# zju3dv/BoxDreamer

Hardware: AMD Instinct MI355X
Metric: poses/s/GPU (5-ref, 224×224, bf16); heatmap max-abs err vs CPU ref (higher is better)
Workload: dtype f16 + e4m3 corrections (BETR q, k columns: f16)

## Files before the change

boxdreamer_amd/csrc/attention.hip:

```cpp
#include "bd_common.h"
#include <type_traits>

#ifdef BD_ATTN_PROBE
__device__ unsigned* bd_attn_probe_buf = nullptr;
extern "C" int bd_attn_probe_set(void* buf) { return (int)hipMemcpyToSymbol(HIP_SYMBOL(bd_attn_probe_buf), &buf, sizeof(buf)); }
#define AP(idx) { const unsigned long long t__ = __builtin_amdgcn_s_memtime(); if ((idx) < 64) probe_ts = (lane == (idx)) ? (unsigned)t__ : probe_ts; }
#else
#define AP(idx) {}
#endif

namespace {

struct AttnArgs {
    const void* qkv; int64_t qkv_plane;
    void* out; int64_t out_plane;
    int batch, seq, heads;
    float scale_log2e;
    const int32_t* q_view;
    int q_len;
    int q_off;
    int out_rows;
};

constexpr int KT = 64;

__device__ __forceinline__ int vswz(int d) { return ((d >> 1) ^ (d >> 4)) & 7; }

__device__ __forceinline__ unsigned pack_lo16(unsigned a, unsigned b) { return __builtin_amdgcn_perm(b, a, 0x05040100u); }
__device__ __forceinline__ unsigned pack_hi16(unsigned a, unsigned b) { return __builtin_amdgcn_perm(b, a, 0x07060302u); }

template <class T, int NS, int HD, int NW, int OUTMODE = 0>
__global__ __launch_bounds__(NW * 64, NS == 1 && HD == 64 ? 3 : 2) void attn_kernel(const AttnArgs p) {
    bd_saturating_conversions();
    typedef typename Op16<T>::vec8 vec8;
    constexpr int NT = NW * 64;
    constexpr int DCH = HD / 8;
    constexpr int KSTRIDE = HD * 2 + 16;
    constexpr int K_BYTES = KT * KSTRIDE;
    constexpr int V_BYTES = HD * 128;
    constexpr int PLANE_BYTES = K_BYTES + V_BYTES;
    constexpr int KCH = KT * DCH;
    constexpr int KCPT = (KCH + NT - 1) / NT;
    constexpr int VMT = (KT / 4) * DCH;
    static_assert(VMT <= NT, "one V micro-tile per thread");
    constexpr int QB = NW * 32;
    constexpr int DM = HD / 32;
    constexpr int KS = HD / 16;
    constexpr int BUF_BYTES = NS * PLANE_BYTES;
    constexpr int NBUF = NS == 1 ? 2 : 1;
    __shared__ __attribute__((aligned(16))) unsigned char lds[NBUF * BUF_BYTES];

    const int tid = threadIdx.x, lane = tid & 63, wid = tid >> 6;
#ifdef BD_ATTN_PROBE
    unsigned probe_ts = 0;
    AP(60)
#endif
    const int lq = lane & 31, lh = lane >> 5;
    const int seq = p.seq, heads = p.heads;
    const int q_len = p.q_len;
    const int nqb = (q_len + QB - 1) / QB;

    int wg;
    {
        const int nwg = gridDim.x, bid = blockIdx.x, xcd = bid & 7, q = nwg >> 3, r = nwg & 7;
        wg = (xcd < r ? xcd * (q + 1) : r * (q + 1) + (xcd - r) * q) + (bid >> 3);
    }
    const int qb = wg % nqb;
    const int bh = wg / nqb;
    const int head = bh % heads, b = bh / heads;

    const int ld = 3 * heads * HD;
    const T* base = (const T*)p.qkv + (int64_t)b * seq * ld + head * HD;
    const T* qbase = base;
    const T* kbase = base + heads * HD;
    const T* vbase = base + 2 * heads * HD;
    const int64_t plane = p.qkv_plane;

    const int q0 = qb * QB + wid * 32;
    const int qbase_row = p.q_view ? p.q_view[b] * q_len : p.q_off;
    int qrow = q0 + lq; qrow = (qrow < q_len ? qrow : q_len - 1) + qbase_row;
    vec8 qf[NS][KS];
#pragma unroll
    for (int s = 0; s < NS; ++s)
#pragma unroll
        for (int ks = 0; ks < KS; ++ks)
            qf[s][ks] = as_vec8<T>(*(const u128*)(qbase + s * plane + (unsigned)(qrow * ld + ks * 16 + lh * 8)));

    int kc_row[KCPT], kc_col[KCPT];
    unsigned kc_off[KCPT];
#pragma unroll
    for (int i = 0; i < KCPT; ++i) {
        const int c = tid + NT * i;
        kc_row[i] = c / DCH;
        kc_col[i] = c % DCH;
        kc_off[i] = (unsigned)(kc_row[i] * ld + kc_col[i] * 8);
    }
    const int vm_kq = tid / DCH, vm_dc = tid % DCH;
    const bool vm_active = tid < VMT;
    const unsigned vm_off = (unsigned)(vm_kq * 4 * ld + vm_dc * 8);
    const bool ragged = (seq % KT) != 0;
    int vdst;
    {
        const int g = vm_kq >> 2, qi = vm_kq & 3;
        const int qp = (qi == 1) ? 2 : (qi == 2 ? 1 : qi);
        vdst = ((g * 2 + (qp >> 1)) << 4) | ((qp & 1) << 3);
    }

    u128 rk[NS][KCPT], rv[NS][4];
    __amdgpu_buffer_rsrc_t rsrc[NS];
    {
        const int bytes = __builtin_amdgcn_readfirstlane(seq * ld * (int)sizeof(T));
#pragma unroll
        for (int s = 0; s < NS; ++s) {
            const uintptr_t a = (uintptr_t)(base + s * plane);
            const unsigned lo = __builtin_amdgcn_readfirstlane((unsigned)a), hi = __builtin_amdgcn_readfirstlane((unsigned)(a >> 32));
            rsrc[s] = __builtin_amdgcn_make_buffer_rsrc((void*)(((uintptr_t)hi << 32) | lo), 0, bytes, 0x00020000);
        }
    }
    const int row_bytes = __builtin_amdgcn_readfirstlane(ld * (int)sizeof(T));
    int k_voff[KCPT];
#pragma unroll
    for (int i = 0; i < KCPT; ++i) k_voff[i] = ((int)kc_off[i] + heads * HD) * (int)sizeof(T);
    const int v_voff = ((int)vm_off + 2 * heads * HD) * (int)sizeof(T);
#define LOAD_TILE(kt)                                                                         \
    _Pragma("unroll") for (int s = 0; s < NS; ++s) {                                          \
        _Pragma("unroll") for (int i = 0; i < KCPT; ++i) {                                    \
            if (KCH % NT == 0 || tid + NT * i < KCH)                                          \
                rk[s][i] = __builtin_bit_cast(u128, __builtin_amdgcn_raw_buffer_load_b128(rsrc[s], k_voff[i], (kt) * KT * row_bytes, 0)); \
        }                                                                                     \
        if (vm_active) {                                                                      \
            _Pragma("unroll") for (int j = 0; j < 4; ++j)                                     \
                rv[s][j] = __builtin_bit_cast(u128, __builtin_amdgcn_raw_buffer_load_b128(rsrc[s], v_voff, ((kt) * KT + j) * row_bytes, 0)); \
        }                                                                                     \
    }
#define STORE_TILE(buf)                                                                        \
    _Pragma("unroll") for (int s = 0; s < NS; ++s) {                                          \
        unsigned char* kl = lds + (buf) * BUF_BYTES + s * PLANE_BYTES;                        \
        unsigned char* vl = kl + K_BYTES;                                                     \
        _Pragma("unroll") for (int i = 0; i < KCPT; ++i)                                      \
            if (KCH % NT == 0 || tid + NT * i < KCH)                                          \
                *(u128*)(kl + kc_row[i] * KSTRIDE + kc_col[i] * 16) = rk[s][i];               \
        if (vm_active) {                                                                      \
            _Pragma("unroll") for (int w = 0; w < 4; ++w) {                                   \
                const unsigned a0 = rv[s][0][w], a1 = rv[s][1][w], a2 = rv[s][2][w], a3 = rv[s][3][w]; \
                const int d = vm_dc * 8 + 2 * w;                                              \
                uint2 lo, hi;                                                                 \
                lo.x = pack_lo16(a0, a1); lo.y = pack_lo16(a2, a3);       \
                hi.x = pack_hi16(a0, a1); hi.y = pack_hi16(a2, a3); \
                *(uint2*)(vl + d * 128 + (vdst ^ (vswz(d) << 4))) = lo;                \
                *(uint2*)(vl + (d + 1) * 128 + (vdst ^ (vswz(d + 1) << 4))) = hi;    \
            }                                                                                 \
        }                                                                                     \
    }

    f32x16 oacc[DM];
#pragma unroll
    for (int i = 0; i < DM; ++i)
#pragma unroll
        for (int r = 0; r < 16; ++r) oacc[i][r] = 0.f;
    float m_run = -INFINITY, l_run = 0.f;
    const float sc = p.scale_log2e;

    const int nt = (seq + KT - 1) / KT;
    LOAD_TILE(0)
    STORE_TILE(0)
    __syncthreads();
    AP(61)
    const bool small_tail = HD == 64 && nt > 1 && seq % KT != 0 && seq % KT <= 16;
    auto tile = [&](const int kt, auto tail_c) {
        constexpr int TAIL = decltype(tail_c)::value;
        constexpr int KMN = TAIL == 2 ? 1 : 2, GN = TAIL == 2 ? 1 : 4;
        if (kt + 1 < nt) { LOAD_TILE(kt + 1) }
        const unsigned char* cur = lds + (NBUF == 2 ? (kt & 1) : 0) * BUF_BYTES;
        if (kt < 7) AP(kt * 8)

        f32x16 sacc[KMN];
#pragma unroll
        for (int km = 0; km < KMN; ++km) {
#pragma unroll
            for (int r = 0; r < 16; ++r) sacc[km][r] = 0.f;
#pragma unroll
            for (int ks = 0; ks < KS; ++ks) {
                vec8 kf[NS];
#pragma unroll
                for (int s = 0; s < NS; ++s)
                    kf[s] = as_vec8<T>(*(const u128*)(cur + s * PLANE_BYTES + (km * 32 + lq) * KSTRIDE + (ks * 2 + lh) * 16));
                if (NS == 2) {
                    sacc[km] = Op16<T>::mfma(kf[NS - 1], qf[0][ks], sacc[km]);
                    sacc[km] = Op16<T>::mfma(kf[0], qf[NS - 1][ks], sacc[km]);
                }
                sacc[km] = Op16<T>::mfma(kf[0], qf[0][ks], sacc[km]);
            }
        }
        if (kt < 7) AP(kt * 8 + 1)
        float tmax = -INFINITY;
        if (TAIL == 2 || (kt + 1) * KT > seq) {
#pragma unroll
            for (int km = 0; km < KMN; ++km)
#pragma unroll
                for (int r = 0; r < 16; ++r) {
                    const int key = kt * KT + km * 32 + (r & 3) + 8 * (r >> 2) + 4 * lh;
                    if (key >= seq) sacc[km][r] = -INFINITY;
                }
        }
#pragma unroll
        for (int km = 0; km < KMN; ++km)
#pragma unroll
            for (int r = 0; r < 16; ++r) tmax = fmaxf(tmax, sacc[km][r]);
        tmax = fmaxf(tmax, __shfl_xor(tmax, 32));
        const float m_new = fmaxf(m_run, tmax);
        if (!__all(m_new == m_run)) {
            const float alpha = __builtin_amdgcn_exp2f((m_run - m_new) * sc);
            l_run *= alpha;
#pragma unroll
            for (int i = 0; i < DM; ++i)
#pragma unroll
                for (int r = 0; r < 16; ++r) oacc[i][r] *= alpha;
            m_run = m_new;
        }
        const float mneg = -m_run * sc;
        float psum = 0.f;
#pragma unroll
        for (int km = 0; km < KMN; ++km)
#pragma unroll
            for (int r = 0; r < 16; ++r) {
                const float pv = __builtin_amdgcn_exp2f(fmaf(sacc[km][r], sc, mneg));
                sacc[km][r] = pv;
                psum += pv;
            }
        l_run += psum;
        if (kt < 7) AP(kt * 8 + 2)

#pragma unroll
        for (int g = 0; g < GN; ++g) {
            vec8 pf[NS];
#pragma unroll
            for (int j = 0; j < 8; ++j) {
                const float pv = sacc[g >> 1][(g & 1) * 8 + j];
                const T hi = from_f32<T>(pv);
                pf[0][j] = hi;
                if (NS == 2) pf[NS - 1][j] = from_f32<T>(pv - to_f32<T>(hi));
            }
#pragma unroll
            for (int dm = 0; dm < DM; ++dm) {
                const int d = dm * 32 + lq;
                vec8 vf[NS];
#pragma unroll
                for (int s = 0; s < NS; ++s)
                    vf[s] = as_vec8<T>(*(const u128*)(cur + s * PLANE_BYTES + K_BYTES + d * 128 +
                                                        (((g * 2 + lh) ^ vswz(d)) << 4)));
                if (NS == 2) {
                    oacc[dm] = Op16<T>::mfma(vf[NS - 1], pf[0], oacc[dm]);
                    oacc[dm] = Op16<T>::mfma(vf[0], pf[NS - 1], oacc[dm]);
                }
                oacc[dm] = Op16<T>::mfma(vf[0], pf[0], oacc[dm]);
            }
        }
        if (kt < 7) AP(kt * 8 + 3)
        if (NBUF == 1) __syncthreads();
        if (kt < 7) AP(kt * 8 + 4)
        if (kt + 1 < nt) { STORE_TILE(NBUF == 2 ? ((kt + 1) & 1) : 0) }
        if (kt < 7) AP(kt * 8 + 5)
        __syncthreads();
        if (kt < 7) AP(kt * 8 + 6)
    };
    for (int kt = 0; kt < nt - (small_tail ? 1 : 0); ++kt) tile(kt, std::integral_constant<int, 0>{});
    if (small_tail) tile(nt - 1, std::integral_constant<int, 2>{});
#undef LOAD_TILE
#undef STORE_TILE

    AP(62)
    const float l_tot = l_run + __shfl_xor(l_run, 32);
    const float inv = 1.0f / l_tot;
    const int q = q0 + lq;
    if (q < q_len) {
        if (OUTMODE == 2) {
            fp8e4* orow = (fp8e4*)p.out + ((int64_t)b * p.out_rows + (p.out_rows == q_len ? 0 : p.q_off) + q) * (heads * HD) + head * HD;
#pragma unroll
            for (int dm = 0; dm < DM; ++dm)
#pragma unroll
                for (int rq = 0; rq < 4; ++rq) {
                    float v4[4];
#pragma unroll
                    for (int j = 0; j < 4; ++j) v4[j] = oacc[dm][rq * 4 + j] * inv;
                    store_cvt<fp8e4, 4>(orow + dm * 32 + 8 * rq + 4 * lh, v4);
                }
        } else if (OUTMODE == 3) {
            const int64_t e0 = ((int64_t)b * p.out_rows + (p.out_rows == q_len ? 0 : p.q_off) + q) * (heads * HD) + head * HD;
#pragma unroll
            for (int dm = 0; dm < DM; ++dm)
#pragma unroll
                for (int rq = 0; rq < 4; ++rq) {
                    float v4[4];
#pragma unroll
                    for (int j = 0; j < 4; ++j) v4[j] = oacc[dm][rq * 4 + j] * inv;
                    f16c8_store4((f16c8*)p.out, p.out_plane, e0 + dm * 32 + 8 * rq + 4 * lh, v4);
                }
        } else if (OUTMODE == 1 || OUTMODE == 4) {
            typedef typename std::conditional<OUTMODE == 1, __bf16, _Float16>::type OT;
            OT* orow = (OT*)p.out + ((int64_t)b * p.out_rows + (p.out_rows == q_len ? 0 : p.q_off) + q) * (heads * HD) + head * HD;
#pragma unroll
            for (int dm = 0; dm < DM; ++dm)
#pragma unroll
                for (int rq = 0; rq < 4; ++rq) {
                    const int d0 = dm * 32 + 8 * rq + 4 * lh;
                    typedef __attribute__((__vector_size__(4 * sizeof(OT)))) OT ovec4;
                    ovec4 hi, lo;
#pragma unroll
                    for (int j = 0; j < 4; ++j) {
                        float h, l;
                        split_hi_lo<OT>(oacc[dm][rq * 4 + j] * inv, h, l);
                        hi[j] = from_f32<OT>(h);
                        lo[j] = from_f32<OT>(l);
                    }
                    *(ovec4*)(orow + d0) = hi;
                    *(ovec4*)(orow + p.out_plane + d0) = lo;
                }
        } else {
            T* orow = (T*)p.out + ((int64_t)b * p.out_rows + (p.out_rows == q_len ? 0 : p.q_off) + q) * (heads * HD) + head * HD;
#pragma unroll
            for (int dm = 0; dm < DM; ++dm)
#pragma unroll
                for (int rq = 0; rq < 4; ++rq) {
                    const int d0 = dm * 32 + 8 * rq + 4 * lh;
                    typedef __attribute__((__vector_size__(4 * sizeof(T)))) T vec4;
                    vec4 hi, lo;
#pragma unroll
                    for (int j = 0; j < 4; ++j) {
                        if (NS == 2) {
                            float h, l;
                            split_hi_lo<T>(oacc[dm][rq * 4 + j] * inv, h, l);
                            hi[j] = from_f32<T>(h);
                            lo[j] = from_f32<T>(l);
                        } else {
                            hi[j] = from_f32<T>(oacc[dm][rq * 4 + j] * inv);
                        }
                    }
                    *(vec4*)(orow + d0) = hi;
                    if (NS == 2) *(vec4*)(orow + p.out_plane + d0) = lo;
                }
        }
    }
#ifdef BD_ATTN_PROBE
    AP(63)
    if (bd_attn_probe_buf && blockIdx.x < 512) bd_attn_probe_buf[((size_t)blockIdx.x * 8 + wid) * 64 + lane] = probe_ts;
#endif
}

template <class T, int HD, int OUTMODE>
__global__ __launch_bounds__(512, 1) void attn_kernel_pp(const AttnArgs p) {
    bd_saturating_conversions();
    typedef typename Op16<T>::vec8 vec8;
    constexpr int NT = 512;
    constexpr int DCH = HD / 8;
    constexpr int KSTRIDE = HD * 2 + 16;
    constexpr int K_BYTES = KT * KSTRIDE;
    constexpr int V_BYTES = HD * 128;
    constexpr int KBUF = 2, VBUF = 4;
    constexpr int VMT = (KT / 4) * DCH;
    static_assert(VMT <= NT, "one V micro-tile per thread");
    constexpr int QB = 256;
    constexpr int DM = HD / 32;
    constexpr int KS = HD / 16;
    constexpr int NPV = 4 * DM, NS_ = 2 * KS, NSLOT = NPV + NS_;
    static_assert(NSLOT >= 22, "softmax schedule below needs 22 slots");
    constexpr bool OUT_VIA_LDS = (OUTMODE == 0 || OUTMODE == 3);
    constexpr int OROW = (OUTMODE == 3) ? HD * 3 : HD * 2;
    constexpr int OSTRIDE = OROW + 16;
    constexpr int RING_BYTES = KBUF * K_BYTES + VBUF * V_BYTES;
    constexpr int LDS_BYTES = (OUT_VIA_LDS && 8 * 32 * OSTRIDE > RING_BYTES) ? 8 * 32 * OSTRIDE : RING_BYTES;
    __shared__ __attribute__((aligned(16))) unsigned char lds[LDS_BYTES];
    unsigned char* const vring = lds;
    unsigned char* const kring = lds + VBUF * V_BYTES;

    const int tid = threadIdx.x, lane = tid & 63;
    const int wid = __builtin_amdgcn_readfirstlane(tid >> 6);
    const int lq = lane & 31, lh = lane >> 5;
    const int seq = p.seq, heads = p.heads;
    const int q_len = p.q_len;
    const int nqb = (q_len + QB - 1) / QB;

    int wg;
    {
        const int nwg = gridDim.x, bid = blockIdx.x, xcd = bid & 7, q = nwg >> 3, r = nwg & 7;
        wg = (xcd < r ? xcd * (q + 1) : r * (q + 1) + (xcd - r) * q) + (bid >> 3);
    }
    const int qb = wg % nqb;
    const int bh = wg / nqb;
    const int head = bh % heads, b = bh / heads;

    const int ld = 3 * heads * HD;
    const T* base = (const T*)p.qkv + (int64_t)b * seq * ld + head * HD;
    const T* kbase = base + heads * HD;
    const T* vbase = base + 2 * heads * HD;

    const int q0 = qb * QB + wid * 32;
    const int qbase_row = p.q_view ? p.q_view[b] * q_len : p.q_off;
    int qrow = q0 + lq; qrow = (qrow < q_len ? qrow : q_len - 1) + qbase_row;
    vec8 qf[KS];
#pragma unroll
    for (int ks = 0; ks < KS; ++ks) qf[ks] = as_vec8<T>(*(const u128*)(base + (unsigned)(qrow * ld + ks * 16 + lh * 8)));

    static_assert(KT * 8 == NT && DCH > 8 && DCH <= 16, "K staging: 8 threads per key row, two pieces each");
    const int kc_row = tid >> 3, kc_col = tid & 7;
    const bool kc_two = kc_col < DCH - 8;
    const int vm_kq = tid / DCH, vm_dc = tid % DCH;
    const bool vm_active = tid < VMT;
    int vdst;
    {
        const int g = vm_kq >> 2, qi = vm_kq & 3;
        const int qp = (qi == 1) ? 2 : (qi == 2 ? 1 : qi);
        vdst = ((g * 2 + (qp >> 1)) << 4) | ((qp & 1) << 3);
    }
    u128 rk[2], rv[4];
    __amdgpu_buffer_rsrc_t rsrc;
    {
        const uintptr_t a = (uintptr_t)base;
        const unsigned lo = __builtin_amdgcn_readfirstlane((unsigned)a), hi = __builtin_amdgcn_readfirstlane((unsigned)(a >> 32));
        rsrc = __builtin_amdgcn_make_buffer_rsrc((void*)(((uintptr_t)hi << 32) | lo), 0, __builtin_amdgcn_readfirstlane(seq * ld * (int)sizeof(T)), 0x00020000);
    }
    const int k_voff = (kc_row * ld + kc_col * 8 + heads * HD) * (int)sizeof(T);
    const int v_voff = (vm_kq * 4 * ld + vm_dc * 8 + 2 * heads * HD) * (int)sizeof(T);
    const int row_bytes = __builtin_amdgcn_readfirstlane(ld * (int)sizeof(T));
    auto load_tile = [&](int kt) {
        const int t_off = kt * KT * row_bytes;
        rk[0] = __builtin_bit_cast(u128, __builtin_amdgcn_raw_buffer_load_b128(rsrc, k_voff, t_off, 0));
        if (kc_two) rk[1] = __builtin_bit_cast(u128, __builtin_amdgcn_raw_buffer_load_b128(rsrc, k_voff + 128, t_off, 0));
        if (vm_active) {
#pragma unroll
            for (int j = 0; j < 4; ++j) rv[j] = __builtin_bit_cast(u128, __builtin_amdgcn_raw_buffer_load_b128(rsrc, v_voff, t_off + j * row_bytes, 0));
        }
    };
    auto store_tile = [&](int kt, int kbi, int vbi) {
        (void)kt;
        unsigned char* kl = kring + kbi * K_BYTES;
        unsigned char* vl = vring + vbi * V_BYTES;
        *(u128*)(kl + kc_row * KSTRIDE + kc_col * 16) = rk[0];
        if (kc_two) *(u128*)(kl + kc_row * KSTRIDE + kc_col * 16 + 128) = rk[1];
        if (vm_active) {
#pragma unroll
            for (int w = 0; w < 4; ++w) {
                const unsigned a0 = rv[0][w], a1 = rv[1][w], a2 = rv[2][w], a3 = rv[3][w];
                const int d = vm_dc * 8 + 2 * w;
                uint2 lo, hi;
                lo.x = pack_lo16(a0, a1); lo.y = pack_lo16(a2, a3);
                hi.x = pack_hi16(a0, a1); hi.y = pack_hi16(a2, a3);
                *(uint2*)(vl + d * 128 + (vdst ^ (vswz(d) << 4))) = lo;
                *(uint2*)(vl + (d + 1) * 128 + (vdst ^ (vswz(d + 1) << 4))) = hi;
            }
        }
    };

    f32x16 oacc[DM];
#pragma unroll
    for (int i = 0; i < DM; ++i)
#pragma unroll
        for (int r = 0; r < 16; ++r) oacc[i][r] = 0.f;
    float m_run = -INFINITY, l_run = 0.f;
    const float sc = p.scale_log2e;
    const int nt = (seq + KT - 1) / KT;
    const f32x16 zero16 = {0.f, 0.f, 0.f, 0.f, 0.f, 0.f, 0.f, 0.f, 0.f, 0.f, 0.f, 0.f, 0.f, 0.f, 0.f, 0.f};

    load_tile(0);
    store_tile(0, 0, 0);
    if (nt > 1) { load_tile(1); store_tile(1, 1, 1); }
    for (int i = tid * 16; i < V_BYTES; i += NT * 16) *(u128*)(vring + (VBUF - 1) * V_BYTES + i) = (u128){0u, 0u, 0u, 0u};
    __syncthreads();

    f32x16 S[2][2];
    vec8 P[4];
#pragma unroll
    for (int g = 0; g < 4; ++g)
#pragma unroll
        for (int j = 0; j < 8; ++j) P[g][j] = from_f32<T>(0.f);
    const unsigned kfrag = (unsigned)(lq * KSTRIDE + lh * 16);
    unsigned vfrag[DM];
#pragma unroll
    for (int dm = 0; dm < DM; ++dm) {
        const int d = dm * 32 + lq;
        vfrag[dm] = (unsigned)(d * 128 + ((lh ^ vswz(d)) << 4));
    }
    {
#pragma unroll
        for (int km = 0; km < 2; ++km)
#pragma unroll
            for (int ks = 0; ks < KS; ++ks) {
                const vec8 kf = as_vec8<T>(*(const u128*)(kring + kfrag + km * 32 * KSTRIDE + ks * 32));
                S[0][km] = Op16<T>::mfma(kf, qf[ks], ks == 0 ? zero16 : S[0][km]);
            }
    }
#ifdef BD_ATTN_PROBE
    unsigned probe_ts = 0;
#endif
#define PP_LOADF(dst, n)                                                                                         \
    {                                                                                                             \
        if ((n) < NPV) {                                                                                          \
            dst = as_vec8<T>(*(const u128*)(vring + ((TI + 3) % VBUF) * V_BYTES + (vfrag[(n) % DM] ^ (unsigned)(((n) / DM) << 5)))); \
        } else {                                                                                                  \
            const int ks_ = ((n) - NPV) / 2, km_ = ((n) - NPV) % 2;          \
            dst = as_vec8<T>(*(const u128*)(kring + ((TI + 1) % KBUF) * K_BYTES + kfrag + km_ * 32 * KSTRIDE + ks_ * 32)); \
        }                                                                                                         \
    }
#define PP_MFMA(n, f)                                                                                            \
    {                                                                                                             \
        if ((n) < NPV) {                                                                                          \
            oacc[(n) % DM] = Op16<T>::mfma(f, P[(n) / DM], oacc[(n) % DM]);                                       \
        } else {                                                                                                  \
            const int ks_ = ((n) - NPV) / 2, km_ = ((n) - NPV) % 2;                                               \
            S[(TI + 1) & 1][km_] = Op16<T>::mfma(f, qf[ks_], ks_ == 0 ? zero16 : S[(TI + 1) & 1][km_]);          \
        }                                                                                                         \
    }
#define PP_ITER(TI_)                                                                                             \
    {                                                                                                             \
        constexpr int TI = (TI_);                                                                                 \
        if (t >= 4 && t < 16) AP((t - 4) * 5)                                                                     \
        const bool stage = t + 2 < nt;                                                                            \
        if (stage) load_tile(t + 2);                                                                              \
        vec8 fr[4];                                                                                               \
        float tmax = -INFINITY, psum = 0.f, mneg = 0.f, alpha = 1.f;                                              \
        bool moved = false;                                                                                       \
        _Pragma("unroll") for (int n = 0; n < 3; ++n) PP_LOADF(fr[n & 3], n)                                      \
        __builtin_amdgcn_sched_barrier(0);                                                                        \
        _Pragma("unroll") for (int n = 0; n < NSLOT; ++n) {                                                       \
            PP_MFMA(n, fr[n & 3])                                                                                 \
            if (n + 3 < NSLOT) PP_LOADF(fr[(n + 3) & 3], n + 3)                                                   \
            if (n < 4) {                                                          \
                _Pragma("unroll") for (int e = n * 8; e < n * 8 + 8; ++e) tmax = fmaxf(tmax, S[TI & 1][e >> 4][e & 15]); \
                asm volatile("" : "+v"(tmax));     \
            } else if (n == 4) {                       \
                float other;          \
                asm volatile("v_mov_b32 %1, %0\n\ts_nop 1\n\tv_permlane32_swap_b32 %0, %1" : "+v"(tmax), "=&v"(other)); \
                tmax = fmaxf(tmax, other);                                                                        \
                const float m_new = fmaxf(m_run, tmax);                                                           \
                moved = !__all(m_new == m_run);                                                                   \
                alpha = __builtin_amdgcn_exp2f((m_run - m_new) * sc);           \
                m_run = m_new;                                                                                    \
                mneg = -m_new * sc;                                                                               \
            } else if (n < 21) {                         \
                _Pragma("unroll") for (int e = (n - 5) * 2; e < (n - 5) * 2 + 2; ++e) {                           \
                    float pv = __builtin_amdgcn_exp2f(fmaf(S[TI & 1][e >> 4][e & 15], sc, mneg));                \
                    asm volatile("" : "+v"(pv));                                                                  \
                    psum += pv;                                                                                   \
                    P[e >> 3][e & 7] = from_f32<T>(pv);                                                           \
                }                                                                                                 \
            }                                                                                                     \
            __builtin_amdgcn_sched_barrier(0);                                                                    \
        }                                                                                                         \
        if (moved) {                        \
            _Pragma("unroll") for (int i = 0; i < DM; ++i)                                                        \
                _Pragma("unroll") for (int r = 0; r < 16; ++r) oacc[i][r] *= alpha;                               \
            l_run *= alpha;                                                                                       \
        }                                                                                                         \
        l_run += psum;                                                                                            \
        if (t >= 4 && t < 16) AP((t - 4) * 5 + 1)                                                                 \
        if (stage) store_tile(t + 2, (TI + 2) % KBUF, (TI + 2) % VBUF);                                           \
        if (t >= 4 && t < 16) AP((t - 4) * 5 + 2)                                                                 \
        __syncthreads();                                                                                          \
        if (t >= 4 && t < 16) AP((t - 4) * 5 + 3)                                                                 \
        ++t;                                                                                                      \
    }
    int t = 0;
    while (t + 4 <= nt) { PP_ITER(0) PP_ITER(1) PP_ITER(2) PP_ITER(3) }
    const int rem = nt - t;
    if (rem > 0) PP_ITER(0)
    if (rem > 1) PP_ITER(1)
    if (rem > 2) PP_ITER(2)
#undef PP_ITER
#undef PP_LOADF
#undef PP_MFMA
#ifdef BD_ATTN_PROBE
    if (bd_attn_probe_buf && blockIdx.x < 512) bd_attn_probe_buf[((size_t)blockIdx.x * 8 + wid) * 64 + lane] = probe_ts;
#endif
    {
        const unsigned char* vcur = vring + ((nt - 1) % VBUF) * V_BYTES;
#pragma unroll
        for (int g = 0; g < 4; ++g)
#pragma unroll
            for (int dm = 0; dm < DM; ++dm) {
                const vec8 vf = as_vec8<T>(*(const u128*)(vcur + (vfrag[dm] ^ (unsigned)(g << 5))));
                oacc[dm] = Op16<T>::mfma(vf, P[g], oacc[dm]);
            }
    }

    const float l_tot = l_run + __shfl_xor(l_run, 32);
    const float inv = 1.0f / l_tot;
    if constexpr (OUT_VIA_LDS) {
        __syncthreads();
        int ln;
        asm volatile("v_mbcnt_lo_u32_b32 %0, -1, 0\n\tv_mbcnt_hi_u32_b32 %0, -1, %0" : "=v"(ln));
        const int lq2 = ln & 31, lh2 = ln >> 5;
        unsigned char* const wl = lds + wid * (32 * OSTRIDE);
        unsigned char* const rowp = wl + lq2 * OSTRIDE;
#pragma unroll
        for (int dm = 0; dm < DM; ++dm)
#pragma unroll
            for (int rq = 0; rq < 4; ++rq) {
                float v4[4];
#pragma unroll
                for (int j = 0; j < 4; ++j) v4[j] = oacc[dm][rq * 4 + j] * inv;
                const int d = dm * 32 + 8 * rq + 4 * lh2;
                if constexpr (OUTMODE == 3) f16c8_store4((f16c8*)rowp, HD, d, v4);
                else store_cvt<T, 4>((T*)rowp + d, v4);
            }
        __builtin_amdgcn_fence(__ATOMIC_RELEASE, "wavefront");
        __builtin_amdgcn_wave_barrier();
        __builtin_amdgcn_fence(__ATOMIC_ACQUIRE, "wavefront");
        constexpr int CPR = OROW / 16, HIC = HD / 8;
        static_assert((32 * CPR) % 64 == 0, "pieces per wave");
        const int64_t row0 = (int64_t)b * p.out_rows + (p.out_rows == q_len ? 0 : p.q_off) + q0;
        unsigned char* const out_hi = (unsigned char*)p.out;
        unsigned char* const out_lo = out_hi + 2 * p.out_plane;
#pragma unroll
        for (int k = 0; k < 32 * CPR / 64; ++k) {
            const int c = ln + 64 * k, r = c / CPR, col = c % CPR;
            if (q0 + r >= q_len) continue;
            const u128 piece = *(const u128*)(wl + r * OSTRIDE + col * 16);
            const int64_t e = (row0 + r) * (heads * HD) + head * HD;
            if (OUTMODE == 3 && col >= HIC) *(u128*)(out_lo + e + (col - HIC) * 16) = piece;
            else *(u128*)(out_hi + 2 * e + col * 16) = piece;
        }
        return;
    }
    const int q = q0 + lq;
    if (q < q_len) {
        const int64_t e0 = ((int64_t)b * p.out_rows + (p.out_rows == q_len ? 0 : p.q_off) + q) * (heads * HD) + head * HD;
#pragma unroll
        for (int dm = 0; dm < DM; ++dm)
#pragma unroll
            for (int rq = 0; rq < 4; ++rq) {
                float v4[4];
#pragma unroll
                for (int j = 0; j < 4; ++j) v4[j] = oacc[dm][rq * 4 + j] * inv;
                const int64_t e = e0 + dm * 32 + 8 * rq + 4 * lh;
                if constexpr (OUTMODE == 2) {
                    store_cvt<fp8e4, 4>((fp8e4*)p.out + e, v4);
                } else if constexpr (OUTMODE == 3) {
                    f16c8_store4((f16c8*)p.out, p.out_plane, e, v4);
                } else if constexpr (OUTMODE == 1 || OUTMODE == 4) {
                    typedef typename std::conditional<OUTMODE == 1, __bf16, _Float16>::type OT;
                    float hi4[4], lo4[4];
#pragma unroll
                    for (int j = 0; j < 4; ++j) split_hi_lo<OT>(v4[j], hi4[j], lo4[j]);
                    store_cvt<OT, 4>((OT*)p.out + e, hi4);
                    store_cvt<OT, 4>((OT*)p.out + p.out_plane + e, lo4);
                } else {
                    store_cvt<T, 4>((T*)p.out + e, v4);
                }
            }
    }
}

template <class T, int HD, int OUTMODE> int launch_pp(const AttnArgs& a, hipStream_t s) {
    const int nqb = (a.q_len + 255) / 256;
    const int slot = bd_trace_open(s, 1, a.batch * a.heads, a.seq, HD);
    hipLaunchKernelGGL((attn_kernel_pp<T, HD, OUTMODE>), dim3(nqb * a.heads * a.batch), dim3(512), 0, s, a);
    bd_trace_close(s, slot);
    BD_CHECK_LAUNCH();
    return BD_OK;
}

template <class T, int NS, int HD, int NW, int OUTMODE = 0> int launch(const AttnArgs& a, hipStream_t s) {
    const int nqb = (a.q_len + NW * 32 - 1) / (NW * 32);
    const int slot = bd_trace_open(s, 1, a.batch * a.heads, a.seq, HD);
    hipLaunchKernelGGL((attn_kernel<T, NS, HD, NW, OUTMODE>), dim3(nqb * a.heads * a.batch), dim3(NW * 64), 0, s, a);
    bd_trace_close(s, slot);
    BD_CHECK_LAUNCH();
    return BD_OK;
}

static thread_local bool g_latency_forms = false;

template <class T, int NS, int OUTMODE = 0> int dispatch(const AttnArgs& a, int head_dim, hipStream_t s) {
    const int waste4 = ((a.q_len + 127) / 128) * 128 - a.q_len, waste3 = ((a.q_len + 95) / 96) * 96 - a.q_len;
    const bool use3 = waste3 < waste4;
    if constexpr (NS == 1) {
        const bool few = g_latency_forms && 4 * ((a.q_len + 255) / 256) * a.heads * a.batch <= 256;
        if (head_dim == 96 && a.q_len % 256 == 0 && a.seq % KT == 0 && !few) return launch_pp<T, 96, OUTMODE>(a, s);
    }
    if (head_dim == 96) return use3 ? launch<T, NS, 96, 3, OUTMODE>(a, s) : launch<T, NS, 96, 4, OUTMODE>(a, s);
    if (head_dim == 64) return use3 ? launch<T, NS, 64, 3, OUTMODE>(a, s) : launch<T, NS, 64, 4, OUTMODE>(a, s);
    return BD_ERR_SHAPE;
}

inline bool sample_bytes_out_of_range(int seq, int heads, int head_dim) {
    return head_dim <= 0 || (int64_t)seq * 3 * heads * head_dim * 2 >= ((int64_t)1 << 31);
}

}

int bd_attention_q_forms(const void* qkv, int64_t qkv_plane, void* out, int64_t out_plane, int batch, int seq, int heads, int head_dim,
                         float scale, const int32_t* q_view, int q_len, int prec, int latency_forms, void* stream) {
    g_latency_forms = latency_forms != 0;
    const int rc = bd_attention_q(qkv, qkv_plane, out, out_plane, batch, seq, heads, head_dim, scale, q_view, q_len, prec, stream);
    g_latency_forms = false;
    return rc;
}

extern "C" int bd_attention_q(const void* qkv, int64_t qkv_plane, void* out, int64_t out_plane, int batch, int seq,
                              int heads, int head_dim, float scale, const int32_t* q_view, int q_len, int prec,
                              void* stream) {
    if (!qkv || !out) return BD_ERR_NULL;
    if (batch <= 0 || seq <= 0 || heads <= 0) return BD_ERR_SHAPE;
    if (q_view ? (q_len <= 0 || q_len > seq || seq % q_len) : (q_len != seq)) return BD_ERR_SHAPE;
    if (sample_bytes_out_of_range(seq, heads, head_dim)) return BD_ERR_SHAPE;
    if (((uintptr_t)qkv & 15) || ((uintptr_t)out & 7)) return BD_ERR_ALIGN;
    AttnArgs a{qkv, qkv_plane, out, out_plane, batch, seq, heads, scale * 1.4426950408889634f, q_view, q_len, 0, q_len};
    hipStream_t s = (hipStream_t)stream;
    switch (prec) {
        case BD_PREC_BF16: return dispatch<__bf16, 1>(a, head_dim, s);
        case BD_PREC_F16: return dispatch<_Float16, 1>(a, head_dim, s);
        case BD_PREC_BF16X3: return dispatch<__bf16, 2>(a, head_dim, s);
        case BD_PREC_F16_OUT_BF16X3: return dispatch<_Float16, 1, 1>(a, head_dim, s);
        case BD_PREC_BF16_OUT_FP8: return dispatch<__bf16, 1, 2>(a, head_dim, s);
        case BD_PREC_F16_OUT_F16C8: return dispatch<_Float16, 1, 3>(a, head_dim, s);
        case BD_PREC_BF16X3_OUT_F16C8: return dispatch<__bf16, 2, 3>(a, head_dim, s);
        case BD_PREC_F16_OUT_F16X3: return dispatch<_Float16, 1, 4>(a, head_dim, s);
        case BD_PREC_BF16X3_OUT_F16X3: return dispatch<__bf16, 2, 4>(a, head_dim, s);
        default: return BD_ERR_DTYPE;
    }
}

#define BD_ATTN_PREC_SWITCH(CALL)                                                       \
    switch (prec) {                                                                     \
        case BD_PREC_BF16: return CALL(__bf16, 1, 0);                                   \
        case BD_PREC_F16: return CALL(_Float16, 1, 0);                                  \
        case BD_PREC_BF16X3: return CALL(__bf16, 2, 0);                                 \
        case BD_PREC_F16_OUT_BF16X3: return CALL(_Float16, 1, 1);                       \
        case BD_PREC_BF16_OUT_FP8: return CALL(__bf16, 1, 2);                           \
        case BD_PREC_F16_OUT_F16C8: return CALL(_Float16, 1, 3);                        \
        case BD_PREC_BF16X3_OUT_F16C8: return CALL(__bf16, 2, 3);                       \
        case BD_PREC_F16_OUT_F16X3: return CALL(_Float16, 1, 4);                        \
        case BD_PREC_BF16X3_OUT_F16X3: return CALL(__bf16, 2, 4);                       \
        default: return BD_ERR_DTYPE;                                                   \
    }

extern "C" int bd_attention_prefix(const void* qkv, int64_t qkv_plane, void* out, int64_t out_plane, int batch, int seq, int heads,
                                   int head_dim, float scale, int n_prefix, int prefix_queries, int prec, void* stream) {
    if (!qkv || !out) return BD_ERR_NULL;
    if (batch <= 0 || seq <= 0 || heads <= 0 || n_prefix <= 0 || n_prefix >= seq) return BD_ERR_SHAPE;
    if (sample_bytes_out_of_range(seq, heads, head_dim)) return BD_ERR_SHAPE;
    if (prefix_queries) return bd_attention_q(qkv, qkv_plane, out, out_plane, batch, seq, heads, head_dim, scale, nullptr, seq, prec, stream);
    if (((uintptr_t)qkv & 15) || ((uintptr_t)out & 7)) return BD_ERR_ALIGN;
    hipStream_t s = (hipStream_t)stream;
    AttnArgs a{qkv, qkv_plane, out, out_plane, batch, seq, heads, scale * 1.4426950408889634f, nullptr, seq - n_prefix, n_prefix, seq};
#define BD_CALL_MAIN(T_, NS_, OM_) dispatch<T_, NS_, OM_>(a, head_dim, s)
    BD_ATTN_PREC_SWITCH(BD_CALL_MAIN)
#undef BD_CALL_MAIN
}

extern "C" int bd_attention(const void* qkv, int64_t qkv_plane, void* out, int64_t out_plane, int batch,
                            int seq, int heads, int head_dim, float scale, int prec, void* stream) {
    return bd_attention_q(qkv, qkv_plane, out, out_plane, batch, seq, heads, head_dim, scale, nullptr, seq, prec, stream);
}
```

Baseline: 767.2.

## Stage V row-major in LDS and read transposed fragments with ds_read_tr16

V tiles were previously loaded as 4-row micro-tiles, permuted in registers with byte-perm instructions and written transposed into LDS. They are now copied straight into LDS in their natural row-major layout, using the same per-thread chunk mapping as K, with an XOR swizzle for HD=64. The PV MFMA operand fragments are gathered with the gfx950 transposing LDS read (ds_read_tr16_b64), two per fragment. This removes the register shuffle and the scattered 8-byte LDS stores from staging, at the cost of twice as many LDS read instructions per V fragment and a new swizzle pattern that may cause bank conflicts.

New measurement: 768.9 (median of 6 runs). Within noise of the previous version (+0.2%).

```diff
diff --git a/boxdreamer_amd/csrc/attention.hip b/boxdreamer_amd/csrc/attention.hip
--- a/boxdreamer_amd/csrc/attention.hip
+++ b/boxdreamer_amd/csrc/attention.hip
@@ -24,10 +24,20 @@
 
 constexpr int KT = 64;
 
-__device__ __forceinline__ int vswz(int d) { return ((d >> 1) ^ (d >> 4)) & 7; }
-
-__device__ __forceinline__ unsigned pack_lo16(unsigned a, unsigned b) { return __builtin_amdgcn_perm(b, a, 0x05040100u); }
-__device__ __forceinline__ unsigned pack_hi16(unsigned a, unsigned b) { return __builtin_amdgcn_perm(b, a, 0x07060302u); }
+template <int HD> __device__ __forceinline__ int vswz(int byte) { return HD == 64 ? byte ^ ((byte >> 2) & 64) : byte; }
+
+__device__ __forceinline__ u128 vt_frag(const unsigned char* lo, const unsigned char* hi) {
+    typedef short v4i16 __attribute__((ext_vector_type(4)));
+    typedef unsigned u32x2 __attribute__((ext_vector_type(2)));
+    const u32x2 a = __builtin_bit_cast(u32x2, __builtin_amdgcn_ds_read_tr16_b64_v4i16((__attribute__((address_space(3))) v4i16*)lo));
+    const u32x2 b = __builtin_bit_cast(u32x2, __builtin_amdgcn_ds_read_tr16_b64_v4i16((__attribute__((address_space(3))) v4i16*)hi));
+    return (u128){a[0], a[1], b[0], b[1]};
+}
+
+template <int HD> __device__ __forceinline__ int vt_lane_base(int lane) {
+    const int q = (lane >> 2) & 3, p = lane & 3, h = lane >> 5, half16 = (lane >> 4) & 1;
+    return 2 * ((4 * h + q) * HD + 16 * half16 + 4 * p);
+}
 
 template <class T, int NS, int HD, int NW, int OUTMODE = 0>
 __global__ __launch_bounds__(NW * 64, NS == 1 && HD == 64 ? 3 : 2) void attn_kernel(const AttnArgs p) {
@@ -37,12 +47,12 @@
     constexpr int DCH = HD / 8;
     constexpr int KSTRIDE = HD * 2 + 16;
     constexpr int K_BYTES = KT * KSTRIDE;
-    constexpr int V_BYTES = HD * 128;
+    constexpr int VROW = HD * 2;
+    constexpr int V_BYTES = KT * VROW;
     constexpr int PLANE_BYTES = K_BYTES + V_BYTES;
     constexpr int KCH = KT * DCH;
     constexpr int KCPT = (KCH + NT - 1) / NT;
-    constexpr int VMT = (KT / 4) * DCH;
-    static_assert(VMT <= NT, "one V micro-tile per thread");
+    static_assert(NT % 32 == 0, "V staging: chunk tid + NT * i keeps chunk tid's swizzle");
     constexpr int QB = NW * 32;
     constexpr int DM = HD / 32;
     constexpr int KS = HD / 16;
@@ -95,18 +105,10 @@
         kc_col[i] = c % DCH;
         kc_off[i] = (unsigned)(kc_row[i] * ld + kc_col[i] * 8);
     }
-    const int vm_kq = tid / DCH, vm_dc = tid % DCH;
-    const bool vm_active = tid < VMT;
-    const unsigned vm_off = (unsigned)(vm_kq * 4 * ld + vm_dc * 8);
+    const int v_st = vswz<HD>(16 * tid);
     const bool ragged = (seq % KT) != 0;
-    int vdst;
-    {
-        const int g = vm_kq >> 2, qi = vm_kq & 3;
-        const int qp = (qi == 1) ? 2 : (qi == 2 ? 1 : qi);
-        vdst = ((g * 2 + (qp >> 1)) << 4) | ((qp & 1) << 3);
-    }
-
-    u128 rk[NS][KCPT], rv[NS][4];
+
+    u128 rk[NS][KCPT], rv[NS][KCPT];
     __amdgpu_buffer_rsrc_t rsrc[NS];
     {
         const int bytes = __builtin_amdgcn_readfirstlane(seq * ld * (int)sizeof(T));
@@ -121,16 +123,14 @@
     int k_voff[KCPT];
 #pragma unroll
     for (int i = 0; i < KCPT; ++i) k_voff[i] = ((int)kc_off[i] + heads * HD) * (int)sizeof(T);
-    const int v_voff = ((int)vm_off + 2 * heads * HD) * (int)sizeof(T);
+    const int v_soff = __builtin_amdgcn_readfirstlane(heads * HD * (int)sizeof(T));
 #define LOAD_TILE(kt)                                                                         \
     _Pragma("unroll") for (int s = 0; s < NS; ++s) {                                          \
         _Pragma("unroll") for (int i = 0; i < KCPT; ++i) {                                    \
-            if (KCH % NT == 0 || tid + NT * i < KCH)                                          \
+            if (KCH % NT == 0 || tid + NT * i < KCH) {                                        \
                 rk[s][i] = __builtin_bit_cast(u128, __builtin_amdgcn_raw_buffer_load_b128(rsrc[s], k_voff[i], (kt) * KT * row_bytes, 0)); \
-        }                                                                                     \
-        if (vm_active) {                                                                      \
-            _Pragma("unroll") for (int j = 0; j < 4; ++j)                                     \
-                rv[s][j] = __builtin_bit_cast(u128, __builtin_amdgcn_raw_buffer_load_b128(rsrc[s], v_voff, ((kt) * KT + j) * row_bytes, 0)); \
+                rv[s][i] = __builtin_bit_cast(u128, __builtin_amdgcn_raw_buffer_load_b128(rsrc[s], k_voff[i], (kt) * KT * row_bytes + v_soff, 0)); \
+            }                                                                                 \
         }                                                                                     \
     }
 #define STORE_TILE(buf)                                                                        \
@@ -138,19 +138,10 @@
         unsigned char* kl = lds + (buf) * BUF_BYTES + s * PLANE_BYTES;                        \
         unsigned char* vl = kl + K_BYTES;                                                     \
         _Pragma("unroll") for (int i = 0; i < KCPT; ++i)                                      \
-            if (KCH % NT == 0 || tid + NT * i < KCH)                                          \
+            if (KCH % NT == 0 || tid + NT * i < KCH) {                                        \
                 *(u128*)(kl + kc_row[i] * KSTRIDE + kc_col[i] * 16) = rk[s][i];               \
-        if (vm_active) {                                                                      \
-            _Pragma("unroll") for (int w = 0; w < 4; ++w) {                                   \
-                const unsigned a0 = rv[s][0][w], a1 = rv[s][1][w], a2 = rv[s][2][w], a3 = rv[s][3][w]; \
-                const int d = vm_dc * 8 + 2 * w;                                              \
-                uint2 lo, hi;                                                                 \
-                lo.x = pack_lo16(a0, a1); lo.y = pack_lo16(a2, a3);       \
-                hi.x = pack_hi16(a0, a1); hi.y = pack_hi16(a2, a3); \
-                *(uint2*)(vl + d * 128 + (vdst ^ (vswz(d) << 4))) = lo;                \
-                *(uint2*)(vl + (d + 1) * 128 + (vdst ^ (vswz(d + 1) << 4))) = hi;    \
+                *(u128*)(vl + v_st + 16 * NT * i) = rv[s][i];                                 \
             }                                                                                 \
-        }                                                                                     \
     }
 
     f32x16 oacc[DM];
@@ -162,6 +153,9 @@
     const float sc = p.scale_log2e;
 
     const int nt = (seq + KT - 1) / KT;
+    int vtr[DM];
+#pragma unroll
+    for (int dm = 0; dm < DM; ++dm) vtr[dm] = vswz<HD>(vt_lane_base<HD>(lane) + 64 * dm);
     LOAD_TILE(0)
     STORE_TILE(0)
     __syncthreads();
@@ -243,12 +237,12 @@
             }
 #pragma unroll
             for (int dm = 0; dm < DM; ++dm) {
-                const int d = dm * 32 + lq;
                 vec8 vf[NS];
 #pragma unroll
-                for (int s = 0; s < NS; ++s)
-                    vf[s] = as_vec8<T>(*(const u128*)(cur + s * PLANE_BYTES + K_BYTES + d * 128 +
-                                                        (((g * 2 + lh) ^ vswz(d)) << 4)));
+                for (int s = 0; s < NS; ++s) {
+                    const unsigned char* vt = cur + s * PLANE_BYTES + K_BYTES + vtr[dm] + g * 16 * VROW;
+                    vf[s] = as_vec8<T>(vt_frag(vt, vt + 8 * VROW));
+                }
                 if (NS == 2) {
                     oacc[dm] = Op16<T>::mfma(vf[NS - 1], pf[0], oacc[dm]);
                     oacc[dm] = Op16<T>::mfma(vf[0], pf[NS - 1], oacc[dm]);
@@ -355,10 +349,9 @@
     constexpr int DCH = HD / 8;
     constexpr int KSTRIDE = HD * 2 + 16;
     constexpr int K_BYTES = KT * KSTRIDE;
-    constexpr int V_BYTES = HD * 128;
+    constexpr int VROW = HD * 2;
+    constexpr int V_BYTES = KT * VROW;
     constexpr int KBUF = 2, VBUF = 4;
-    constexpr int VMT = (KT / 4) * DCH;
-    static_assert(VMT <= NT, "one V micro-tile per thread");
     constexpr int QB = 256;
     constexpr int DM = HD / 32;
     constexpr int KS = HD / 16;
@@ -401,18 +394,10 @@
 #pragma unroll
     for (int ks = 0; ks < KS; ++ks) qf[ks] = as_vec8<T>(*(const u128*)(base + (unsigned)(qrow * ld + ks * 16 + lh * 8)));
 
-    static_assert(KT * 8 == NT && DCH > 8 && DCH <= 16, "K staging: 8 threads per key row, two pieces each");
+    static_assert(KT * 8 == NT && DCH > 8 && DCH <= 16, "K / V staging: 8 threads per key row, two pieces each");
     const int kc_row = tid >> 3, kc_col = tid & 7;
     const bool kc_two = kc_col < DCH - 8;
-    const int vm_kq = tid / DCH, vm_dc = tid % DCH;
-    const bool vm_active = tid < VMT;
-    int vdst;
-    {
-        const int g = vm_kq >> 2, qi = vm_kq & 3;
-        const int qp = (qi == 1) ? 2 : (qi == 2 ? 1 : qi);
-        vdst = ((g * 2 + (qp >> 1)) << 4) | ((qp & 1) << 3);
-    }
-    u128 rk[2], rv[4];
+    u128 rk[2], rv[2];
     __amdgpu_buffer_rsrc_t rsrc;
     {
         const uintptr_t a = (uintptr_t)base;
@@ -420,15 +405,16 @@
         rsrc = __builtin_amdgcn_make_buffer_rsrc((void*)(((uintptr_t)hi << 32) | lo), 0, __builtin_amdgcn_readfirstlane(seq * ld * (int)sizeof(T)), 0x00020000);
     }
     const int k_voff = (kc_row * ld + kc_col * 8 + heads * HD) * (int)sizeof(T);
-    const int v_voff = (vm_kq * 4 * ld + vm_dc * 8 + 2 * heads * HD) * (int)sizeof(T);
     const int row_bytes = __builtin_amdgcn_readfirstlane(ld * (int)sizeof(T));
+    const int v_soff = __builtin_amdgcn_readfirstlane(heads * HD * (int)sizeof(T));
+    const int v_st = kc_row * VROW + kc_col * 16;
     auto load_tile = [&](int kt) {
         const int t_off = kt * KT * row_bytes;
         rk[0] = __builtin_bit_cast(u128, __builtin_amdgcn_raw_buffer_load_b128(rsrc, k_voff, t_off, 0));
-        if (kc_two) rk[1] = __builtin_bit_cast(u128, __builtin_amdgcn_raw_buffer_load_b128(rsrc, k_voff + 128, t_off, 0));
-        if (vm_active) {
-#pragma unroll
-            for (int j = 0; j < 4; ++j) rv[j] = __builtin_bit_cast(u128, __builtin_amdgcn_raw_buffer_load_b128(rsrc, v_voff, t_off + j * row_bytes, 0));
+        rv[0] = __builtin_bit_cast(u128, __builtin_amdgcn_raw_buffer_load_b128(rsrc, k_voff, t_off + v_soff, 0));
+        if (kc_two) {
+            rk[1] = __builtin_bit_cast(u128, __builtin_amdgcn_raw_buffer_load_b128(rsrc, k_voff + 128, t_off, 0));
+            rv[1] = __builtin_bit_cast(u128, __builtin_amdgcn_raw_buffer_load_b128(rsrc, k_voff + 128, t_off + v_soff, 0));
         }
     };
     auto store_tile = [&](int kt, int kbi, int vbi) {
@@ -436,18 +422,10 @@
         unsigned char* kl = kring + kbi * K_BYTES;
         unsigned char* vl = vring + vbi * V_BYTES;
         *(u128*)(kl + kc_row * KSTRIDE + kc_col * 16) = rk[0];
-        if (kc_two) *(u128*)(kl + kc_row * KSTRIDE + kc_col * 16 + 128) = rk[1];
-        if (vm_active) {
-#pragma unroll
-            for (int w = 0; w < 4; ++w) {
-                const unsigned a0 = rv[0][w], a1 = rv[1][w], a2 = rv[2][w], a3 = rv[3][w];
-                const int d = vm_dc * 8 + 2 * w;
-                uint2 lo, hi;
-                lo.x = pack_lo16(a0, a1); lo.y = pack_lo16(a2, a3);
-                hi.x = pack_hi16(a0, a1); hi.y = pack_hi16(a2, a3);
-                *(uint2*)(vl + d * 128 + (vdst ^ (vswz(d) << 4))) = lo;
-                *(uint2*)(vl + (d + 1) * 128 + (vdst ^ (vswz(d + 1) << 4))) = hi;
-            }
+        *(u128*)(vl + v_st) = rv[0];
+        if (kc_two) {
+            *(u128*)(kl + kc_row * KSTRIDE + kc_col * 16 + 128) = rk[1];
+            *(u128*)(vl + v_st + 128) = rv[1];
         }
     };
 
@@ -474,12 +452,7 @@
 #pragma unroll
         for (int j = 0; j < 8; ++j) P[g][j] = from_f32<T>(0.f);
     const unsigned kfrag = (unsigned)(lq * KSTRIDE + lh * 16);
-    unsigned vfrag[DM];
-#pragma unroll
-    for (int dm = 0; dm < DM; ++dm) {
-        const int d = dm * 32 + lq;
-        vfrag[dm] = (unsigned)(d * 128 + ((lh ^ vswz(d)) << 4));
-    }
+    const unsigned vfrag = (unsigned)vt_lane_base<HD>(lane);
     {
 #pragma unroll
         for (int km = 0; km < 2; ++km)
@@ -495,7 +468,8 @@
 #define PP_LOADF(dst, n)                                                                                         \
     {                                                                                                             \
         if ((n) < NPV) {                                                                                          \
-            dst = as_vec8<T>(*(const u128*)(vring + ((TI + 3) % VBUF) * V_BYTES + (vfrag[(n) % DM] ^ (unsigned)(((n) / DM) << 5)))); \
+            const unsigned char* vt_ = vring + ((TI + 3) % VBUF) * V_BYTES + vfrag + ((n) % DM) * 64 + ((n) / DM) * 16 * VROW; \
+            dst = as_vec8<T>(vt_frag(vt_, vt_ + 8 * VROW));                                                      \
         } else {                                                                                                  \
             const int ks_ = ((n) - NPV) / 2, km_ = ((n) - NPV) % 2;          \
             dst = as_vec8<T>(*(const u128*)(kring + ((TI + 1) % KBUF) * K_BYTES + kfrag + km_ * 32 * KSTRIDE + ks_ * 32)); \
@@ -572,12 +546,13 @@
     if (bd_attn_probe_buf && blockIdx.x < 512) bd_attn_probe_buf[((size_t)blockIdx.x * 8 + wid) * 64 + lane] = probe_ts;
 #endif
     {
-        const unsigned char* vcur = vring + ((nt - 1) % VBUF) * V_BYTES;
+        const unsigned char* vcur = vring + ((nt - 1) % VBUF) * V_BYTES + vfrag;
 #pragma unroll
         for (int g = 0; g < 4; ++g)
 #pragma unroll
             for (int dm = 0; dm < DM; ++dm) {
-                const vec8 vf = as_vec8<T>(*(const u128*)(vcur + (vfrag[dm] ^ (unsigned)(g << 5))));
+                const unsigned char* vt = vcur + dm * 64 + g * 16 * VROW;
+                const vec8 vf = as_vec8<T>(vt_frag(vt, vt + 8 * VROW));
                 oacc[dm] = Op16<T>::mfma(vf, P[g], oacc[dm]);
             }
     }
```
